# PinataFarms/DAD-3DHeads

Measured on AMD Instinct MI355X. Metric: images/sec (FLAME decode + 445-lmk projection), batch 64 @ 256^2, higher is better.
Workload: dtype f32

## Files before the change

### dad-3dheads_amd/_lib.py

```python
from __future__ import annotations

import ctypes as C
import os

_HERE = os.path.dirname(os.path.abspath(__file__))
LIB_PATH = os.environ.get("DAD3D_LIB_PATH") or os.path.join(_HERE, "libdad3d_hip.so")

OK, E_INVALID, E_HIP, E_UNSUPPORTED, E_NOMEM = range(5)
ZERO_ROTATION, TO_2D, MUTATE_PARAMS, FLIP_Z, COMPAT_CROSS_B3 = 0x1, 0x2, 0x4, 0x8, 0x10
NORMAL_ACCUMULATE = 0x1
PLAN_GET_NORMAL, PLAN_PHONG, PLAN_RENDER = 0, 1, 2
FORM_REFUSED, FORM_TABLE, FORM_LDS, FORM_GLOBAL = 0, 1, 2, 3
TEX_INDEX_CORNER, TEX_INDEX_REFERENCE = 0, 1
DTYPE_F32, DTYPE_U8 = 0, 1
EVAL_SELF_EXCLUDE, EVAL_MAX_K, EVAL_MAX_HEAD, EVAL_MAX_ANCHORS = 0x1, 8, 4096, 8
HEATMAP_RAW, HEATMAP_UINT8, HEATMAP_FLOAT = 0, 1, 2
OBJ_MAX_LINE_BYTES, OBJ_FLAG_NONFINITE, OBJ_FLAG_LARGE = 71, 0x1, 0x2
JSON_MAX_NUMBER_BYTES, JSON_MAX_LITERAL_BYTES, JSON_FLAG_NONFINITE = 23, 64, 0x1
JSON_PARSE_TILE_BYTES, JSON_PARSE_RECORD_INTS = 4096, 6
(JSON_PARSE_FLAG_GRAMMAR, JSON_PARSE_FLAG_DIGITS, JSON_PARSE_FLAG_BIG_INT, JSON_PARSE_FLAG_SUBNORMAL, JSON_PARSE_FLAG_OVERFLOW,
 JSON_PARSE_FLAG_AMBIGUOUS) = 0x1, 0x2, 0x4, 0x8, 0x10, 0x20
(ANNOTATION_FLAG_GRAMMAR, ANNOTATION_FLAG_KEYS, ANNOTATION_FLAG_SHAPE, ANNOTATION_FLAG_NUMBER, ANNOTATION_FLAG_STRING,
 ANNOTATION_FLAG_RANGE) = 0x1, 0x2, 0x4, 0x8, 0x10, 0x20
ANNOTATION_MAX_BACKSLASH_RUN, ANNOTATION_MAX_WORD_BYTES, ANNOTATION_MAX_KEY_BYTES, ANNOTATION_MAX_KEYS = 64, 32, 64, 128
# ... 40 lines not shown
        ("specular_exp", C.c_float),
        ("color_ambient", C.c_float * 3),
        ("color_directional", C.c_float * 3),
        ("light_pos", C.c_float * 3),
        ("view_pos", C.c_float * 3),
    ]


_P, _I, _U, _F = C.c_void_p, C.c_int, C.c_uint, C.c_float
SIGNATURES = {
    "dad3d_last_error": (C.c_char_p, []),
    "dad3d_clear_error": (None, []),
    "dad3d_version": (_I, []),
    "dad3d_build_info": (C.c_char_p, []),
    "dad3d_device_count": (_I, []),
    "dad3d_flame_create": (_I, [C.POINTER(FlameModelC), C.POINTER(FlameConstsC), _F, _I, C.POINTER(_P)]),
    "dad3d_flame_destroy": (None, [_P]),
    "dad3d_flame_fork": (_I, [_P, C.POINTER(_P)]),
    "dad3d_flame_num_params": (_I, [_P]),
    "dad3d_flame_num_verts": (_I, [_P]),
    "dad3d_flame_set_landmarks": (_I, [_P, _P, _I]),
    "dad3d_flame_num_landmarks": (_I, [_P]),
    "dad3d_flame_num_landmark_vertices": (_I, [_P]),
    "dad3d_flame_decode": (_I, [_P, _P, _I, _U, _P, _P, _P, _P, _P]),
    "dad3d_flame_decode_posed": (_I, [_P, _P, _I, _U, _P, _P, _P, _P]),
    "dad3d_flame_decode_backward": (_I, [_P, _I, _U, _P, _P, _P, _P, _P, _P, _P]),
    "dad3d_flame_grad_inputs": (_I, [_P, _P, _I, _P, _P]),
    "dad3d_flame_num_chain_inputs": (_I, [_P]),
    "dad3d_flame_pose_chain": (_I, [_P, _P, _I, _P, _P, _P]),
    "dad3d_flame_pose_chain_backward": (_I, [_P, _P, _I, _P, _P, _P, _P]),
    "dad3d_flame_decode_host": (_I, [_P, _P, _I, _U, _P, _P, _P, _P]),
    "dad3d_flame_readjust_params": (_I, [_P, _P, _I, _P, _F, _F, _F, _P]),
    "dad3d_flame_profile_begin": (_I, [_P, _P]),
    "dad3d_flame_profile_end": (_I, [_P, _P, C.POINTER(C.c_double), C.POINTER(_I)]),
    "dad3d_flame_select_kernel": (_I, [_P, _I]),
    "dad3d_flame_handoff_timeouts": (_I, [_P, C.POINTER(C.c_uint)]),
    "dad3d_flame_debug_trace": (_I, [_P, _P, C.c_uint64]),
    "dad3d_flame_debug_trace_entries": (C.c_uint64, [_P, _I]),
    "dad3d_mesh_create": (_I, [_P, _I, _I, _I, C.POINTER(_P)]),
    "dad3d_mesh_destroy": (None, [_P]),
    "dad3d_mesh_get_normal": (_I, [_P, _P, _P, _I, _U, _P]),
    "dad3d_mesh_get_tri_normal": (_I, [_P, _P, _P, _I, _I, _P]),
    "dad3d_mesh_get_ver_normal": (_I, [_P, _P, _P, _I, _U, _P]),
    "dad3d_mesh_rasterize": (_I, [_P, _P, _P, _P, _P, _I, _I, _I, _I, _F, _I, _P]),
    "dad3d_mesh_rasterize_triangles": (_I, [_P, _P, _P, _P, _P, _I, _I, _I, _P]),
    "dad3d_mesh_phong_light": (_I, [_P, _P, _P, _P, _I, C.POINTER(LightC), _P]),
# ... 89 lines not shown
```

### dad-3dheads_amd/csrc/capi.cpp

```cpp
#include <algorithm>
#include <cmath>
#include <cstdlib>
#include <cstring>
#include <memory>
#include <mutex>

#include "common.hpp"

namespace dad3d {

static thread_local std::string g_last_error;

void set_error(const char* fmt, ...) {
    char buf[1024];
    va_list ap;
    va_start(ap, fmt);
    vsnprintf(buf, sizeof buf, fmt, ap);
    va_end(ap);
    g_last_error = buf;
}

template <typename T>
static dad3d_status upload(T** dst, const std::vector<T>& src) {
    *dst = nullptr;
// ... 427 lines not shown

static dad3d_status ensure_basis_f16(FlameConsts* c, hipStream_t s) {
    std::lock_guard<std::mutex> lock(c->f16_mu);
    if (c->d_bpack_f16) return DAD3D_OK;
    hipStreamCaptureStatus capture = hipStreamCaptureStatusNone;
    if (s != nullptr) (void)hipStreamIsCapturing(s, &capture);
    DAD3D_REQUIRE(capture == hipStreamCaptureStatusNone, "the first fp16-split decode of a model builds its basis planes: run it once before capturing a graph");
    const size_t bytes = (size_t)c->n_tiles_pipe * kPipeKGroups * 4 * 64 * 4 * sizeof(float);
    float* d = nullptr;
    DAD3D_HIP_TRY(hipMalloc(reinterpret_cast<void**>(&d), bytes));
    dad3d_status st = launch_split_basis_f16(c->d_bpack_pipe, d, c->n_tiles_pipe, c->split_b_scale, s);
    if (st == DAD3D_OK && hipStreamSynchronize(s) != hipSuccess) {
        set_error("ensure_basis_f16: hipStreamSynchronize failed");
        st = DAD3D_E_HIP;
    }
    if (st) {
        (void)hipFree(d);
        return st;
    }
    c->d_bpack_f16 = d;
    return DAD3D_OK;
}

static dad3d_status ensure_split_scratch(dad3d_flame* h, int n_phase, hipStream_t s) {
    if (n_phase <= h->split_cap) return DAD3D_OK;
    hipStreamCaptureStatus capture = hipStreamCaptureStatusNone;
    if (s != nullptr) (void)hipStreamIsCapturing(s, &capture);
    DAD3D_REQUIRE(capture == hipStreamCaptureStatusNone,
                  "the first split-kernel decode of a handle (and the first at a larger batch) allocates: run it once before capturing a graph");
    if (h->d_split_a) h->split_retired.push_back(h->d_split_a);
    h->d_split_a = nullptr, h->split_cap = 0;
    DAD3D_HIP_TRY(hipMalloc(reinterpret_cast<void**>(&h->d_split_a), (size_t)n_phase * kSplitBlockBytes));
    DAD3D_HIP_TRY(hipMemsetAsync(h->d_split_a, 0, (size_t)n_phase * kSplitBlockBytes, s));
    h->split_cap = n_phase;
    return DAD3D_OK;
}

static int resolve_kernel(const dad3d_flame* h, int pinned, int batch, unsigned flags, bool posed) {
    const bool pipe_covers = h->c->d_bpack_pipe && !posed && !(flags & (DAD3D_COMPAT_CROSS_B3 | DAD3D_ZERO_ROTATION)) &&
                             (size_t)batch * h->n_verts * 12 < ((size_t)1 << 31) && (size_t)batch * std::max(h->lmk->n, 1) * 8 < ((size_t)1 << 31);
    if (pinned == DAD3D_KERNEL_TWO_ROLE || (pinned == DAD3D_KERNEL_AUTO && !pipe_covers)) return DAD3D_KERNEL_TWO_ROLE;
    if (pipe_covers) return pinned == DAD3D_KERNEL_AUTO ? DAD3D_KERNEL_PIPELINED : pinned;
    set_error("dad3d_flame_decode: the %s kernel does not cover this launch (model, flags or output size)",
              pinned == DAD3D_KERNEL_PIPELINED ? "pipelined" : "split");
    return -1;
}
// ... 3 lines not shown
    DAD3D_REQUIRE(h, "dad3d_flame_decode: null handle");
    DAD3D_REQUIRE(batch >= 0, "dad3d_flame_decode: negative batch");
    if (batch == 0) return DAD3D_OK;
    DAD3D_REQUIRE(params, "dad3d_flame_decode: null params");
    DAD3D_REQUIRE(!((flags & DAD3D_FLIP_Z) && (flags & DAD3D_TO_2D)), "DAD3D_FLIP_Z needs a 3-component projection");
    DAD3D_REQUIRE(!(posed && (flags & DAD3D_COMPAT_CROSS_B3)), "DAD3D_COMPAT_CROSS_B3 is inference-only (dad3d_flame_decode_posed refuses it)");
    DeviceGuard guard(h->device);
    hipStream_t s = static_cast<hipStream_t>(stream);
    const int pinned = h->kernel_choice >= 0 ? h->kernel_choice : decode_kernel_choice();
    const int kernel = resolve_kernel(h, pinned, batch, flags, posed != nullptr);
    if (kernel < 0) return DAD3D_E_UNSUPPORTED;
    const LandmarkList& L = *h->lmk;
    const int n_lmk = (lmk_xy || lmk_px) ? L.n : 0;

    const bool on_sub = L.sub && !verts3d && !proj && n_lmk && !h->d_trace && pinned != DAD3D_KERNEL_PIPELINED;
    FlameConsts* c = on_sub ? L.sub.get() : h->c.get();
    const float4* vtab = on_sub ? L.d_sub_vtab : L.d_vtab;
    const int n_verts = on_sub ? L.sub_verts : h->n_verts;

    dad3d_status st;
    if (kernel == DAD3D_KERNEL_SPLIT_BF16 || kernel == DAD3D_KERNEL_SPLIT_F16) {
        DAD3D_REQUIRE(!h->d_trace, "dad3d_flame_decode: the split kernels have no trace stamps");
        const int n_phase = (batch + kSplitRows - 1) / kSplitRows;
        st = ensure_split_scratch(h, n_phase, s);
        if (!st && kernel == DAD3D_KERNEL_SPLIT_F16) st = ensure_basis_f16(c, s);
        if (!st && kernel == DAD3D_KERNEL_SPLIT_F16 && L.sub) st = ensure_basis_f16(L.sub.get(), s);
        if (st) return st;
        SplitArgs sa{};
        sa.params = params;
        sa.bpack = c->d_bpack_pipe;
        sa.bpack_f16 = c->d_bpack_f16;
        sa.vtab = vtab;
        sa.lmk_next = L.d_next;
        sa.verts3d = verts3d;
        sa.proj = proj;
        sa.lmk_xy = lmk_xy;
        sa.lmk_px = lmk_px;
        sa.aplanes = h->d_split_a;
        sa.b_scale = c->split_b_scale;
        sa.n_params = h->lay.n_params;
        sa.batch = batch;
        sa.n_phase = n_phase;
        sa.n_tiles = c->n_tiles_pipe;
        split_chunking(sa.n_tiles, n_phase, &sa.n_chunks, &sa.phases_per_chunk);
        sa.n_verts = n_verts;
        sa.n_lmk = n_lmk;
        sa.image_size = h->image_size;
        sa.flags = flags & 0xFFu;
        st = launch_flame_decode_split(sa, kernel, s);
    } else if (kernel == DAD3D_KERNEL_PIPELINED) {
        DAD3D_REQUIRE(!h->d_trace || h->trace_capacity >= trace_entries_pipe(h), "dad3d_flame_decode: the trace buffer holds %llu entries, "
                      "this launch stamps %llu (dad3d_flame_debug_trace_entries)", (unsigned long long)h->trace_capacity,
                      (unsigned long long)trace_entries_pipe(h));
        PipeArgs pa{};
        pa.params = params;
        pa.bpack = c->d_bpack_pipe;
        pa.vtab = vtab;
        pa.lmk_next = L.d_next;
        pa.verts3d = verts3d;
        pa.proj = proj;
        pa.lmk_xy = lmk_xy;
        pa.lmk_px = lmk_px;
        pa.trace = h->d_trace;
        pa.n_params = h->lay.n_params;
        pa.batch = batch;
        pa.n_half = (batch + kPipeHalf - 1) / kPipeHalf;
        pa.n_tiles = c->n_tiles_pipe;
// ... 101 lines not shown
    if (!st) fail(hipDeviceSynchronize(), "hipDeviceSynchronize");
    if (!st && (flags & DAD3D_MUTATE_PARAMS)) fail(hipMemcpy(params, d_par, n_par * sizeof(float), hipMemcpyDeviceToHost), "hipMemcpy");
    if (!st && n_v) fail(hipMemcpy(verts3d, d_v, n_v * sizeof(float), hipMemcpyDeviceToHost), "hipMemcpy");
    if (!st && n_p) fail(hipMemcpy(proj, d_p, n_p * sizeof(float), hipMemcpyDeviceToHost), "hipMemcpy");
    if (!st && n_lx) fail(hipMemcpy(lmk_xy, d_lx, n_lx * sizeof(float), hipMemcpyDeviceToHost), "hipMemcpy");
    if (!st && n_lp) fail(hipMemcpy(lmk_px, d_lp, n_lp * sizeof(int32_t), hipMemcpyDeviceToHost), "hipMemcpy");
    (void)hipFree(d);
    return st;
}

dad3d_status dad3d_flame_readjust_params(dad3d_flame* h, float* params, int batch, const float* pads_scale,
                                         float pad_left, float pad_top, float scale, void* stream) {
    DAD3D_REQUIRE(h && batch >= 0, "dad3d_flame_readjust_params: bad argument");
    if (batch == 0) return DAD3D_OK;
    DAD3D_REQUIRE(params, "dad3d_flame_readjust_params: null params");
    DeviceGuard guard(h->device);
    return launch_readjust(params, batch, h->lay, pads_scale, pad_left, pad_top, scale, h->image_size,
                           static_cast<hipStream_t>(stream));
}

dad3d_status dad3d_flame_select_kernel(dad3d_flame* h, int which) {
    DAD3D_REQUIRE(h && which >= DAD3D_KERNEL_AUTO && which <= DAD3D_KERNEL_SPLIT_F16, "dad3d_flame_select_kernel: bad argument");
    h->kernel_choice = which;
    return DAD3D_OK;
}

dad3d_status dad3d_flame_handoff_timeouts(dad3d_flame* h, unsigned* count) {
    DAD3D_REQUIRE(h && count, "null argument");
    DeviceGuard guard(h->device);
    DAD3D_HIP_TRY(hipDeviceSynchronize());
    DAD3D_HIP_TRY(hipMemcpy(count, h->d_sync + 1, sizeof(unsigned), hipMemcpyDeviceToHost));
    return DAD3D_OK;
}

uint64_t dad3d_flame_debug_trace_entries(const dad3d_flame* h, int batch) {
    if (!h || batch <= 0) return 0;
    return std::max(trace_entries_two_role(h, batch), trace_entries_pipe(h));
}

dad3d_status dad3d_flame_debug_trace(dad3d_flame* h, unsigned long long* device_buffer, uint64_t capacity) {
    DAD3D_REQUIRE(h, "null handle");
    h->d_trace = device_buffer;
    h->trace_capacity = device_buffer ? capacity : 0;
    return DAD3D_OK;
}

// ... 1314 lines not shown
```

### dad-3dheads_amd/csrc/common.hpp

```cpp
#pragma once

#include <hip/hip_runtime.h>

#include <atomic>
#include <cstdarg>
#include <cstdint>
#include <cstdio>
#include <string>
#include <vector>

#include "../../include/dad3d.h"

namespace dad3d {

void set_error(const char* fmt, ...);

#define DAD3D_HIP_TRY(expr)                                                                      \
    do {                                                                                         \
        hipError_t e__ = (expr);                                                                 \
        if (e__ != hipSuccess) {                                                                 \
            ::dad3d::set_error("%s failed: %s (%s:%d)", #expr, hipGetErrorString(e__), __FILE__, \
                               __LINE__);                                                        \
            return DAD3D_E_HIP;                                                                  \
        }                                                                                        \
// ... 121 lines not shown
    float* params;
    const float* bpack;
    const float* bpack_f16;
    const float4* vtab;
    const int* lmk_next;
    float* verts3d;
    float* proj;
    float* lmk_xy;
    int32_t* lmk_px;
    char* aplanes;
    float b_scale;
    int n_params, batch, n_phase, n_tiles, n_verts, n_lmk;
    int n_chunks, phases_per_chunk;
    float image_size;
    unsigned flags;
};
inline void split_chunking(int n_tiles, int n_phase, int* n_chunks, int* phases_per_chunk) {
    *n_chunks = 1, *phases_per_chunk = n_phase;
    const int max_chunks = 256 / n_tiles;
    if (max_chunks < 2 || n_phase < 2) return;
    *phases_per_chunk = (n_phase + max_chunks - 1) / max_chunks;
    *n_chunks = (n_phase + *phases_per_chunk - 1) / *phases_per_chunk;
}
dad3d_status launch_flame_decode_split(const SplitArgs& a, int form, hipStream_t s);
float split_basis_scale(float max_abs);
dad3d_status launch_split_basis_f16(const float* bpack, float* bpack_f16, int n_tiles, float scale, hipStream_t s);
size_t flame_decode_split_lds_bytes();

constexpr int kBackwardConsts = 72;
struct BackwardArgs {
    const float* weights8;
    const float* consts;
    const float* posed;
    const float* g_verts3d;
    const float* g_proj;
    float* g_posed;
    float* g_consts;
    float* partials;
    int batch, n_verts, nsplit;
    float image_size;
    unsigned flags;
};
dad3d_status launch_flame_backward(const BackwardArgs& a, hipStream_t s);
constexpr int kBackwardMaxSplit = 8;

constexpr int kGradChunk = 256;
// ... 376 lines not shown
```

### dad-3dheads_amd/csrc/flame_decode_split.hip

```cpp
#pragma clang fp contract(off)
#include "common.hpp"
#include "flame_math.hpp"
#include "flame_pipe_epilogue.hpp"

#ifndef DAD3D_SPLIT_ABLATE
#define DAD3D_SPLIT_ABLATE 0
#endif

#ifndef DAD3D_SPLIT_FIN_PRIO
#define DAD3D_SPLIT_FIN_PRIO 1
#endif

namespace dad3d {

namespace {

using namespace pipe;

typedef __bf16 bf16x8 __attribute__((ext_vector_type(8)));
typedef _Float16 f16x8 __attribute__((ext_vector_type(8)));
typedef float f32x8 __attribute__((ext_vector_type(8)));

constexpr int TV = kPipeTileVerts;
constexpr int kJawCol = 3 * TV;
// ... 34 lines not shown
    static constexpr int c_off = a_off + 3 * PLN;
    static constexpr int o_off = c_off + 8 * CST;
    static constexpr int v_off = o_off + 2 * 2 * QB * OS * 4;
    static constexpr int total = v_off + TV * 16;
    static_assert(total <= 160 * 1024 && c_off % 1024 == 0 && o_off % 16 == 0 && v_off % 16 == 0, "LDS budget of one CU");
};

__device__ __forceinline__ void phase_barrier() {
    asm volatile("s_waitcnt lgkmcnt(0)\n\ts_barrier" ::: "memory");
}

template <class V>
__device__ __forceinline__ f32x8 peel(f32x8 r, V& plane) {
    plane = __builtin_convertvector(r, V);
    return r - __builtin_convertvector(plane, f32x8);
}

__device__ __forceinline__ void glds_1k(const char* gsrc_lane, char* lds_base) {
    __builtin_amdgcn_global_load_lds((const __attribute__((address_space(1))) void*)gsrc_lane, (__attribute__((address_space(3))) void*)lds_base, 16, 0, 0);
}

}

template <class S>
__global__ __launch_bounds__(256) void split_params_kernel(SplitArgs a) {
    constexpr int PLN = S::PLN, BLK = S::PLN + CST;
    const int b = blockIdx.x, t = threadIdx.x, P = a.n_params;
    if (DAD3D_SPLIT_ABLATE & 2048) return;
    const bool live = b < a.batch;
    float* prow = a.params + (size_t)min(b, a.batch - 1) * P;
    char* blk = a.aplanes + (size_t)(b / QB) * BLK;
    char* row = blk + (size_t)(b % QB) * RS;
    if ((DAD3D_SPLIT_ABLATE & 4096) && *reinterpret_cast<const volatile unsigned*>(row) != 0u) return;
    float D[9] = {0.f, 0.f, 0.f, 0.f, 0.f, 0.f, 0.f, 0.f, 0.f};
    if (t >= 192) {
        const float jaw[3] = {prow[kNumBeta], prow[kNumBeta + 1], prow[kNumBeta + 2]};
        rodrigues_minus_identity_lean(jaw, D);
    }
    if (t < 208) {
        const int k0 = 2 * t;
        float x = 0.f, y = 0.f;
        if (k0 < kNumBeta) x = prow[k0], y = prow[k0 + 1];
        const float tail[16] = {D[0], D[1], D[2], D[3], D[4], D[5], D[6], D[7], D[8], 1.0f, 0.f, 0.f, 0.f, 0.f, 0.f, 0.f};
#pragma unroll
        for (int i = 0; i < 8; ++i)
            if (t - kNumBeta / 2 == i) x = tail[2 * i], y = tail[2 * i + 1];
        if (!live || (DAD3D_SPLIT_ABLATE & 16384)) x = y = 0.f;
        const int g = k0 >> 5, h = (k0 >> 4) & 1, q = (k0 >> 2) & 3, i = k0 & 3;
        const int pos = 32 * g + 8 * q + 4 * h + i;
        float rx = x * S::kScaleA, ry = y * S::kScaleA;
#pragma unroll
        for (int pl = 0; pl < S::NPL; ++pl) {
            const typename S::elem hx = (typename S::elem)rx, hy = (typename S::elem)ry;
            rx = rx - (float)hx, ry = ry - (float)hy;
            const unsigned packed = (unsigned)__builtin_bit_cast(unsigned short, hx) | ((unsigned)__builtin_bit_cast(unsigned short, hy) << 16);
            *reinterpret_cast<unsigned*>(row + (size_t)pl * QB * RS + 2 * pos) = packed;
        }
    } else if (t < 208 + 4 * S::NPL) {
        const int pl = (t - 208) >> 2, w = (t - 208) & 3;
        *reinterpret_cast<unsigned*>(row + (size_t)pl * QB * RS + 832 + 4 * w) = 0u;
    } else if (t == 255 && !(DAD3D_SPLIT_ABLATE & 8192)) {
        float* c = reinterpret_cast<float*>(blk + PLN + (size_t)(b % QB) * 96);
        *reinterpret_cast<float4*>(c) = float4{D[0], D[1], D[2], D[3]};
        *reinterpret_cast<float4*>(c + 4) = float4{D[4], D[5], D[6], D[7]};
        c[8] = D[8];
    }
    if (t == 0 && !(DAD3D_SPLIT_ABLATE & 8192)) {
        const float rot6[6] = {prow[403], prow[404], prow[405], prow[406], prow[407], prow[408]};
        const float sp1 = prow[412] + 1.0f, tx = prow[409], ty = prow[410];
        float G[9];
        rot6_to_matrix_lean(rot6, G);
        const float s = sp1 < 1e-8f ? 1e-8f : sp1;
        float* c = reinterpret_cast<float*>(blk + PLN + (size_t)(b % QB) * 96);
        c[9] = G[0], c[10] = G[1], c[11] = G[2];
        *reinterpret_cast<float4*>(c + 12) = float4{G[3], G[4], G[5], G[6]};
        const float hh = a.image_size * 0.5f;
        *reinterpret_cast<float4*>(c + 16) = float4{G[7], G[8], s * hh, (tx + 1.0f) * hh};
        *reinterpret_cast<float4*>(c + 20) = float4{(ty + 1.0f) * hh, hh, 0.f, 0.f};
        if ((a.flags & DAD3D_MUTATE_PARAMS) && live) prow[kNumBeta + 11] = 0.0f;
    }
}

template <class S, bool TO2D, bool WB>
__global__ __launch_bounds__(64 * (5 + S::kFinishers), (5 + S::kFinishers + 3) / 4) void flame_decode_split_kernel(SplitArgs a) {
    typedef typename S::vec8 vec8;
    constexpr int NPL = S::NPL, PLN = S::PLN, BLK = S::PLN + CST;
    extern __shared__ __attribute__((aligned(1024))) char smem[];
    char* abuf = smem + Lds<S>::a_off;
    char* cring = smem + Lds<S>::c_off;
    float* otile = reinterpret_cast<float*>(smem + Lds<S>::o_off);
    float4* vt_lds = reinterpret_cast<float4*>(smem + Lds<S>::v_off);

    const int tid = threadIdx.x, lane = tid & 63;
    const int wave = __builtin_amdgcn_readfirstlane(tid >> 6);
    const int n_work = a.n_tiles * a.n_chunks;
    const int xcd = blockIdx.x & 7, slot = blockIdx.x >> 3, big = n_work & 7, per = n_work >> 3;
    const int work = xcd < big ? xcd * (per + 1) + slot : big * (per + 1) + (xcd - big) * per + slot;
    const int tile = work / a.n_chunks, chunk = work - tile * a.n_chunks, v0 = tile * TV;
    const int pb = chunk * a.phases_per_chunk;
    const int NP = min(a.phases_per_chunk, a.n_phase - pb), B = a.batch;
    if (NP <= 0) return;

    if (wave == 4) {
        auto stage = [&](int p) {
            const char* src = a.aplanes + (size_t)(pb + p) * BLK + 16 * lane;
            char* dst = abuf + (p % 3) * PLN;
#if defined(DAD3D_SPLIT_NO_GLDS)
#pragma unroll 1
            for (int i0 = 0; i0 < PLN / 1024; i0 += 8) {
                f32x4 v[8];
#pragma unroll
                for (int i = 0; i < 8; ++i) v[i] = *reinterpret_cast<const f32x4*>(src + 1024 * (i0 + i));
#pragma unroll
                for (int i = 0; i < 8; ++i) *reinterpret_cast<f32x4*>(dst + 1024 * (i0 + i) + 16 * lane) = v[i];
            }
            for (int i = 0; i < CST / 1024; ++i)
                *reinterpret_cast<f32x4*>(cring + (p & 7) * CST + 1024 * i + 16 * lane) = *reinterpret_cast<const f32x4*>(src + PLN + 1024 * i);
#else
#pragma unroll 8
            for (int i = 0; i < PLN / 1024; ++i) glds_1k(src + 1024 * i, dst + 1024 * i);
#pragma unroll
            for (int i = 0; i < CST / 1024; ++i) glds_1k(src + PLN + 1024 * i, cring + (p & 7) * CST + 1024 * i);
#endif
        };
        constexpr int kStageOps = PLN / 1024 + CST / 1024;
        static_assert(kStageOps <= 63, "vmcnt is a 6-bit counter");
        if (lane < TV) vt_lds[lane] = a.vtab[min(v0 + lane, a.n_verts - 1)];
        asm volatile("s_waitcnt vmcnt(0)" ::: "memory");
        stage(0);
        if (NP > 1) {
            stage(1);
            asm volatile("s_waitcnt vmcnt(%0)" ::"n"(kStageOps) : "memory");
        } else {
            asm volatile("s_waitcnt vmcnt(0)" ::: "memory");
        }
        phase_barrier();
#pragma unroll 1
        for (int p = 0; p < NP; ++p) {
            if (p + 2 < NP && (!(DAD3D_SPLIT_ABLATE & 2) || p < 1)) {
                stage(p + 2);
                asm volatile("s_waitcnt vmcnt(%0)" ::"n"(kStageOps) : "memory");
            } else {
                asm volatile("s_waitcnt vmcnt(0)" ::: "memory");
            }
            phase_barrier();
        }
        phase_barrier();
        return;
    }
    const unsigned nl = (unsigned)a.n_lmk;
    EpiCtx cx;
// ... 29 lines not shown
    struct Call {
        float4 k0, k1, k2, k3, k4, k5;
        float j0[3], j1[3], e0[3], e1[3];
    };
    auto load_call = [&](int q, const Geo& g, Call& t) {
        const float4* cp = reinterpret_cast<const float4*>(cring + (q & 7) * CST + g.cp_off);
        t.k0 = cp[0], t.k1 = cp[1], t.k2 = cp[2], t.k3 = cp[3], t.k4 = cp[4], t.k5 = cp[5];
        const float* ot = otile + (q & 1) * (2 * QB * OS);
#pragma unroll
        for (int k = 0; k < 3; ++k) {
            t.j0[k] = ot[g.jt_off + k], t.j1[k] = ot[QB * OS + g.jt_off + k];
            t.e0[k] = ot[g.ot_off + k], t.e1[k] = ot[QB * OS + g.ot_off + k];
        }
    };
    auto math_call = [&](const Geo& g, const Call& t) {
        if (DAD3D_SPLIT_ABLATE & 512) return VertexOut{t.e0[0] + t.k0.x, t.e0[1] + t.k1.x, t.e0[2] + t.k2.x, t.e1[0] + t.k3.x + t.j0[0], t.e1[1] + t.k4.x + t.j0[1], t.e1[2] + t.k5.x + t.j1[0]};
        return vertex_math_folded(cx, t.k0, t.k1, t.k2, t.k3, t.k4, t.k5, t.j0[0] + t.j1[0], t.j0[1] + t.j1[1], t.j0[2] + t.j1[2], t.e0[0] + t.e1[0],
                                  t.e0[1] + t.e1[1], t.e0[2] + t.e1[2], g.vt.x, g.vt.y);
    };
    auto store_call = [&](int q, const Geo& g, const VertexOut& o) {
        const int b = (pb + q) * QB + g.i;
        const bool live = b < B && g.vlive && !((DAD3D_SPLIT_ABLATE & 256) && o.ox != 12345.678f);
        const unsigned row0 = (unsigned)((pb + q) * QB) * (unsigned)a.n_verts;
        vertex_store_at<TO2D, WB ? 0 : DAD3D_PIPE_STORE_AUX>(cx, rs3, rsp, o, __float_as_int(g.vt.z), __float_as_int(g.vt.w), live && a.verts3d != nullptr, live && a.proj != nullptr,
                              live && nl > 0 && __float_as_int(g.vt.z) >= 0, g.off3 + row0 * 12u, g.offp + row0 * kPB, (unsigned)b * nl);
    };
    auto finish_one = [&](int q, const Geo& g) {
        Call t;
        load_call(q, g, t);
        store_call(q, g, math_call(g, t));
    };
    auto finish_two = [&](int q, const Geo& ga, const Geo& gb) {
        Call ta, tb;
        load_call(q, ga, ta);
        load_call(q, gb, tb);
        const VertexOut oa = math_call(ga, ta), ob = math_call(gb, tb);
        store_call(q, ga, oa);
        store_call(q, gb, ob);
    };

    if (wave > 4) {
        const int fj = wave - 5;
        __builtin_amdgcn_s_setprio(DAD3D_SPLIT_FIN_PRIO);
        phase_barrier();
        constexpr bool kTwoCalls = S::kFinishers == 3;
        const Geo ga = make_geo(fj), gb = make_geo(kTwoCalls && fj < 2 ? fj + 3 : fj);
#pragma unroll 1
        for (int p = 0; p < NP; ++p) {
            if (p >= 2 && !(DAD3D_SPLIT_ABLATE & 1)) {
                if (kTwoCalls && fj < 2) finish_two(p - 2, ga, gb);
                else finish_one(p - 2, ga);
            }
            phase_barrier();
        }
        if (NP >= 2 && !(DAD3D_SPLIT_ABLATE & 1)) finish_one(NP - 2, ga);
        phase_barrier();
        if (!(DAD3D_SPLIT_ABLATE & 1)) finish_one(NP - 1, ga);
        return;
    }

    const int kh = wave >> 1, ch = wave & 1, c0 = 2 * ch + kh, c1 = 2 * ch + 1 - kh, gbase = 6 * kh;
    const float4* bsrc = reinterpret_cast<const float4*>(S::kScaled ? a.bpack_f16 : a.bpack) + (size_t)tile * kPipeKGroups * 256 + lane;
    float4 raw[6][2][2], rawt[2][2];
#pragma unroll
    for (int sl = 0; sl < 6; ++sl)
#pragma unroll
        for (int cb = 0; cb < 2; ++cb)
#pragma unroll
            for (int h = 0; h < 2; ++h) {
                raw[sl][cb][h] = bsrc[(size_t)((2 * (gbase + sl) + h) * 4 + (cb ? c1 : c0)) * 64];
                __builtin_amdgcn_sched_barrier(0);
            }
#pragma unroll
    for (int cb = 0; cb < 2; ++cb)
#pragma unroll
// ... 76 lines not shown
    const long long clk0 = clock64(), wall0 = wall_clock64();
#endif
    read_frags(0, gbase, af);
    if constexpr (S::kScaled) {
#pragma unroll
        for (int sl = 0; sl < 6; ++sl) planes(raw[sl][0][0], raw[sl][0][1], bp[sl][0]), planes(raw[sl][1][0], raw[sl][1][1], bp[sl][1]);
        planes(rawt[0][0], rawt[0][1], bt[0]), planes(rawt[1][0], rawt[1][1], bt[1]);
#pragma unroll 1
        for (int p = 0; p < NP; ++p) phase(p, std::false_type{});
    } else {
        phase(0, std::true_type{});
#pragma unroll 1
        for (int p = 1; p < NP; ++p) phase(p, std::false_type{});
    }
    if (S::kFinishers == 3 && wave < 2 && !(DAD3D_SPLIT_ABLATE & 1)) {
        const Geo g = make_geo(3 + wave);
        if (NP >= 2) finish_one(NP - 2, g);
        phase_barrier();
        finish_one(NP - 1, g);
        return;
    }
    phase_barrier();
#if defined(DAD3D_SPLIT_CLOCKS)
    if (tile == 17 && tid == 130) {
        unsigned* cnt = reinterpret_cast<unsigned*>(a.aplanes + PLN + 1536);
        const unsigned n = atomicAdd(cnt, 1u);
        const long long dc = clock64() - clk0, dw = wall_clock64() - wall0;
        if ((n & 255u) == 255u) printf("CLK n_phase %d cycles %lld ticks %lld MHz %.0f cycles/phase %.0f\n", NP, dc, dw, (double)dc / (dw * 10.0) * 1e3, (double)dc / NP);
    }
#endif
}

__global__ __launch_bounds__(256) void split_basis_f16_kernel(const float4* src, float4* dst, int n_tiles, float scale) {
    const size_t i = (size_t)blockIdx.x * 256 + threadIdx.x;
    const size_t n = (size_t)n_tiles * kSplitKGroups * 256;
    if (i >= n) return;
    const size_t t = i / (kSplitKGroups * 256), g = (i / 256) % kSplitKGroups, r = i % 256;
    const size_t i0 = (t * kPipeKGroups + 2 * g) * 256 + r, i1 = i0 + 256;
    const float4 lo = src[i0], hi = src[i1];
    float e[8] = {lo.x, lo.y, lo.z, lo.w, hi.x, hi.y, hi.z, hi.w};
    f16x8 h1, h2;
#pragma unroll
    for (int k = 0; k < 8; ++k) {
        const float x = e[k] * scale;
        h1[k] = (_Float16)x;
        h2[k] = (_Float16)(x - (float)h1[k]);
    }
    dst[i0] = __builtin_bit_cast(float4, h1), dst[i1] = __builtin_bit_cast(float4, h2);
}

dad3d_status launch_split_basis_f16(const float* bpack, float* bpack_f16, int n_tiles, float scale, hipStream_t s) {
    static_assert(kPipeKGroups == 2 * kSplitKGroups, "two MFMA groups of 16 k per 16-bit group of 32");
    const size_t n = (size_t)n_tiles * kSplitKGroups * 256;
    hipLaunchKernelGGL(split_basis_f16_kernel, dim3((unsigned)((n + 255) / 256)), dim3(256), 0, s, reinterpret_cast<const float4*>(bpack),
                       reinterpret_cast<float4*>(bpack_f16), n_tiles, scale);
    DAD3D_HIP_TRY(hipGetLastError());
    return DAD3D_OK;
}

size_t flame_decode_split_lds_bytes() { return (size_t)Lds<Bf16x3>::total; }

namespace {
template <class S>
dad3d_status launch_split(const SplitArgs& a, hipStream_t s, PerDeviceOnce& attr_done) {
    const int dev = PerDeviceOnce::current();
    const size_t lds = (size_t)Lds<S>::total;
    if (!attr_done.done(dev)) {
        for (const void* k : {reinterpret_cast<const void*>(&flame_decode_split_kernel<S, true, false>),
                              reinterpret_cast<const void*>(&flame_decode_split_kernel<S, false, false>),
                              reinterpret_cast<const void*>(&flame_decode_split_kernel<S, true, true>),
                              reinterpret_cast<const void*>(&flame_decode_split_kernel<S, false, true>)})
            DAD3D_HIP_TRY(hipFuncSetAttribute(k, hipFuncAttributeMaxDynamicSharedMemorySize, (int)lds));
        attr_done.set(dev);
    }
    hipLaunchKernelGGL(split_params_kernel<S>, dim3(a.n_phase * kSplitRows), dim3(256), 0, s, a);
    const bool to2d = (a.flags & DAD3D_TO_2D) || !a.proj, wb = a.batch >= S::kWriteBackFrom;
    const dim3 grid(a.n_tiles * a.n_chunks), block(64 * (5 + S::kFinishers));
    if (to2d && wb) hipLaunchKernelGGL((flame_decode_split_kernel<S, true, true>), grid, block, lds, s, a);
    else if (to2d) hipLaunchKernelGGL((flame_decode_split_kernel<S, true, false>), grid, block, lds, s, a);
    else if (wb) hipLaunchKernelGGL((flame_decode_split_kernel<S, false, true>), grid, block, lds, s, a);
    else hipLaunchKernelGGL((flame_decode_split_kernel<S, false, false>), grid, block, lds, s, a);
    DAD3D_HIP_TRY(hipGetLastError());
    return DAD3D_OK;
}
}

dad3d_status launch_flame_decode_split(const SplitArgs& a, int form, hipStream_t s) {
    static PerDeviceOnce attr_bf16, attr_f16;
    if (form == DAD3D_KERNEL_SPLIT_F16) return launch_split<F16x2>(a, s, attr_f16);
    return launch_split<Bf16x3>(a, s, attr_bf16);
}

float split_basis_scale(float max_abs) {
    float s = 1.0f;
    while (s < 16777216.0f && max_abs * (s * 2.0f) <= 16384.0f) s *= 2.0f;
    return s;
}

}
```

### include/dad3d.h

```cpp
#ifndef DAD3D_H_
#define DAD3D_H_

#include <stddef.h>
#include <stdint.h>

#ifndef DAD3D_EXPORT
#define DAD3D_EXPORT __attribute__((visibility("default")))
#endif

#ifdef __cplusplus
extern "C" {
#endif

#define DAD3D_VERSION 100

typedef enum dad3d_status {
    DAD3D_OK = 0,
    DAD3D_E_INVALID = 1,
    DAD3D_E_HIP = 2,
    DAD3D_E_UNSUPPORTED = 3,
    DAD3D_E_NOMEM = 4
} dad3d_status;

DAD3D_EXPORT const char* dad3d_last_error(void);
// ... 18 lines not shown
typedef struct dad3d_flame_consts {
    int32_t shape, expression, jaw, rotation, eyeballs, neck, translation, scale;
} dad3d_flame_consts;

typedef struct dad3d_flame dad3d_flame;

#define DAD3D_ZERO_ROTATION 0x1u
#define DAD3D_TO_2D 0x2u
#define DAD3D_MUTATE_PARAMS 0x4u
#define DAD3D_FLIP_Z 0x8u
#define DAD3D_COMPAT_CROSS_B3 0x10u

DAD3D_EXPORT dad3d_status dad3d_flame_create(const dad3d_flame_model* model, const dad3d_flame_consts* consts, float image_size,
                                int device, dad3d_flame** out);
DAD3D_EXPORT void dad3d_flame_destroy(dad3d_flame* h);
DAD3D_EXPORT dad3d_status dad3d_flame_fork(dad3d_flame* parent, dad3d_flame** out);

DAD3D_EXPORT int dad3d_flame_num_params(const dad3d_flame* h);
DAD3D_EXPORT int dad3d_flame_num_verts(const dad3d_flame* h);

DAD3D_EXPORT dad3d_status dad3d_flame_set_landmarks(dad3d_flame* h, const int64_t* indices, int n);
DAD3D_EXPORT int dad3d_flame_num_landmarks(const dad3d_flame* h);
DAD3D_EXPORT int dad3d_flame_num_landmark_vertices(const dad3d_flame* h);

DAD3D_EXPORT dad3d_status dad3d_flame_decode(dad3d_flame* h, float* params, int batch, unsigned flags, float* verts3d, float* proj,
                                float* lmk_xy, int32_t* lmk_px, void* stream);

DAD3D_EXPORT dad3d_status dad3d_flame_decode_posed(dad3d_flame* h, float* params, int batch, unsigned flags, float* verts3d, float* proj,
                                      float* posed, void* stream);

DAD3D_EXPORT dad3d_status dad3d_flame_decode_backward(dad3d_flame* h, int batch, unsigned flags, const float* consts, const float* posed,
                                         const float* grad_verts3d, const float* grad_proj, float* grad_posed,
                                         float* grad_consts, void* stream);

#define DAD3D_GRAD_INPUTS_MAX_BATCH 96
DAD3D_EXPORT dad3d_status dad3d_flame_grad_inputs(dad3d_flame* h, const float* grad_posed, int batch, float* grad_inputs, void* stream);

DAD3D_EXPORT int dad3d_flame_num_chain_inputs(const dad3d_flame* h);
DAD3D_EXPORT dad3d_status dad3d_flame_pose_chain(dad3d_flame* h, const float* params, int batch, float* inputs, float* consts, void* stream);
DAD3D_EXPORT dad3d_status dad3d_flame_pose_chain_backward(dad3d_flame* h, const float* params, int batch, const float* grad_inputs,
                                             const float* grad_consts, float* grad_params, void* stream);

DAD3D_EXPORT dad3d_status dad3d_flame_decode_host(dad3d_flame* h, float* params, int batch, unsigned flags, float* verts3d,
                                     float* proj, float* lmk_xy, int32_t* lmk_px);

DAD3D_EXPORT dad3d_status dad3d_flame_readjust_params(dad3d_flame* h, float* params, int batch, const float* pads_scale,
// ... 245 lines not shown
```

Baseline: 5.030 million.

## Fuse param splitting into split decode kernel for landmark-only small-batch path

For landmark-only decodes on the landmark subset with at most two phases per workgroup, the separate split_params_kernel launch is removed. Each decode workgroup now reads the raw parameters and builds the bf16/f16 plane images and per-row constants itself, using the staging and finisher waves as producers. This cuts one kernel launch and the global round trip through the A-plane scratch, at the cost of every tile redundantly recomputing the parameter split. It is on by default and can be turned off with an environment variable, and a plan query API is added.

Result: no change. 5.037 million (median of 4 runs) (+0.1%).

```diff
diff --git a/dad-3dheads_amd/_lib.py b/dad-3dheads_amd/_lib.py
--- a/dad-3dheads_amd/_lib.py
+++ b/dad-3dheads_amd/_lib.py
@@ -86,6 +86,7 @@
     "dad3d_flame_set_landmarks": (_I, [_P, _P, _I]),
     "dad3d_flame_num_landmarks": (_I, [_P]),
     "dad3d_flame_num_landmark_vertices": (_I, [_P]),
+    "dad3d_flame_landmark_plan": (_I, [_P, _I, C.POINTER(_I), C.POINTER(_I), C.POINTER(_I), C.POINTER(_I), C.POINTER(_I)]),
     "dad3d_flame_decode": (_I, [_P, _P, _I, _U, _P, _P, _P, _P, _P]),
     "dad3d_flame_decode_posed": (_I, [_P, _P, _I, _U, _P, _P, _P, _P]),
     "dad3d_flame_decode_backward": (_I, [_P, _I, _U, _P, _P, _P, _P, _P, _P, _P]),
diff --git a/dad-3dheads_amd/csrc/capi.cpp b/dad-3dheads_amd/csrc/capi.cpp
--- a/dad-3dheads_amd/csrc/capi.cpp
+++ b/dad-3dheads_amd/csrc/capi.cpp
@@ -473,6 +473,14 @@
     return DAD3D_OK;
 }
 
+static bool split_lmk_one_launch() {
+    static const bool on = [] {
+        const char* e = getenv("DAD3D_SPLIT_LMK_ONE_LAUNCH");
+        return !(e && e[0] == '0');
+    }();
+    return on;
+}
+
 static dad3d_status ensure_split_scratch(dad3d_flame* h, int n_phase, hipStream_t s) {
     if (n_phase <= h->split_cap) return DAD3D_OK;
     hipStreamCaptureStatus capture = hipStreamCaptureStatusNone;
@@ -522,7 +530,10 @@
     if (kernel == DAD3D_KERNEL_SPLIT_BF16 || kernel == DAD3D_KERNEL_SPLIT_F16) {
         DAD3D_REQUIRE(!h->d_trace, "dad3d_flame_decode: the split kernels have no trace stamps");
         const int n_phase = (batch + kSplitRows - 1) / kSplitRows;
-        st = ensure_split_scratch(h, n_phase, s);
+        int n_chunks = 1, phases_per_chunk = n_phase;
+        split_chunking(c->n_tiles_pipe, n_phase, &n_chunks, &phases_per_chunk);
+        const bool one_launch = on_sub && phases_per_chunk <= kSplitOneLaunchPhases && split_lmk_one_launch();
+        st = one_launch ? DAD3D_OK : ensure_split_scratch(h, n_phase, s);
         if (!st && kernel == DAD3D_KERNEL_SPLIT_F16) st = ensure_basis_f16(c, s);
         if (!st && kernel == DAD3D_KERNEL_SPLIT_F16 && L.sub) st = ensure_basis_f16(L.sub.get(), s);
         if (st) return st;
@@ -536,13 +547,13 @@
         sa.proj = proj;
         sa.lmk_xy = lmk_xy;
         sa.lmk_px = lmk_px;
-        sa.aplanes = h->d_split_a;
+        sa.aplanes = one_launch ? nullptr : h->d_split_a;
         sa.b_scale = c->split_b_scale;
         sa.n_params = h->lay.n_params;
         sa.batch = batch;
         sa.n_phase = n_phase;
         sa.n_tiles = c->n_tiles_pipe;
-        split_chunking(sa.n_tiles, n_phase, &sa.n_chunks, &sa.phases_per_chunk);
+        sa.n_chunks = n_chunks, sa.phases_per_chunk = phases_per_chunk;
         sa.n_verts = n_verts;
         sa.n_lmk = n_lmk;
         sa.image_size = h->image_size;
@@ -690,6 +701,29 @@
 dad3d_status dad3d_flame_select_kernel(dad3d_flame* h, int which) {
     DAD3D_REQUIRE(h && which >= DAD3D_KERNEL_AUTO && which <= DAD3D_KERNEL_SPLIT_F16, "dad3d_flame_select_kernel: bad argument");
     h->kernel_choice = which;
+    return DAD3D_OK;
+}
+
+dad3d_status dad3d_flame_landmark_plan(dad3d_flame* h, int batch, int* kernel, int* tiles, int* chunks, int* rows_per_chunk, int* launches) {
+    DAD3D_REQUIRE(h && batch > 0 && kernel && tiles && chunks && rows_per_chunk && launches, "dad3d_flame_landmark_plan: bad argument");
+    const int pinned = h->kernel_choice >= 0 ? h->kernel_choice : decode_kernel_choice();
+    const int k = resolve_kernel(h, pinned, batch, 0u, false);
+    if (k < 0) return DAD3D_E_UNSUPPORTED;
+    const LandmarkList& L = *h->lmk;
+    const bool on_sub = L.sub && L.n && !h->d_trace && pinned != DAD3D_KERNEL_PIPELINED && k != DAD3D_KERNEL_TWO_ROLE;
+    *kernel = k;
+    *tiles = k == DAD3D_KERNEL_TWO_ROLE ? h->n_tiles : on_sub ? L.sub->n_tiles_pipe : h->c->n_tiles_pipe;
+    *chunks = 1, *rows_per_chunk = batch, *launches = 1;
+    if (k == DAD3D_KERNEL_SPLIT_BF16 || k == DAD3D_KERNEL_SPLIT_F16) {
+        int ppc = 0;
+        split_chunking(*tiles, (batch + kSplitRows - 1) / kSplitRows, chunks, &ppc);
+        *rows_per_chunk = ppc * kSplitRows;
+        *launches = on_sub && ppc <= kSplitOneLaunchPhases && split_lmk_one_launch() ? 1 : 2;
+    } else if (k == DAD3D_KERNEL_PIPELINED && !h->d_trace) {
+        int chunk_half = 0, wg = 0;
+        pipe_chunking(*tiles, (batch + kPipeHalf - 1) / kPipeHalf, &chunk_half, chunks, &wg);
+        if (chunk_half > 0) *rows_per_chunk = chunk_half * kPipeHalf;
+    }
     return DAD3D_OK;
 }
 
diff --git a/dad-3dheads_amd/csrc/common.hpp b/dad-3dheads_amd/csrc/common.hpp
--- a/dad-3dheads_amd/csrc/common.hpp
+++ b/dad-3dheads_amd/csrc/common.hpp
@@ -167,6 +167,7 @@
     *phases_per_chunk = (n_phase + max_chunks - 1) / max_chunks;
     *n_chunks = (n_phase + *phases_per_chunk - 1) / *phases_per_chunk;
 }
+constexpr int kSplitOneLaunchPhases = 2;
 dad3d_status launch_flame_decode_split(const SplitArgs& a, int form, hipStream_t s);
 float split_basis_scale(float max_abs);
 dad3d_status launch_split_basis_f16(const float* bpack, float* bpack_f16, int n_tiles, float scale, hipStream_t s);
diff --git a/dad-3dheads_amd/csrc/flame_decode_split.hip b/dad-3dheads_amd/csrc/flame_decode_split.hip
--- a/dad-3dheads_amd/csrc/flame_decode_split.hip
+++ b/dad-3dheads_amd/csrc/flame_decode_split.hip
@@ -80,6 +80,79 @@
 
 }
 
+__device__ __forceinline__ void load_jaw(const float* prow, float (&jaw)[3]) {
+    jaw[0] = prow[kNumBeta], jaw[1] = prow[kNumBeta + 1], jaw[2] = prow[kNumBeta + 2];
+}
+__device__ __forceinline__ void load_pose(const float* prow, float (&v)[9]) {
+#pragma unroll
+    for (int i = 0; i < 8; ++i) v[i] = prow[403 + i];
+    v[8] = prow[412];
+}
+__device__ __forceinline__ void jaw_feature(const float (&jaw)[3], float (&D)[9]) {
+    rodrigues_minus_identity_lean(jaw, D);
+}
+__device__ __forceinline__ void store_jaw_constants(const float (&D)[9], float* c) {
+    *reinterpret_cast<float4*>(c) = float4{D[0], D[1], D[2], D[3]};
+    *reinterpret_cast<float4*>(c + 4) = float4{D[4], D[5], D[6], D[7]};
+    c[8] = D[8];
+}
+__device__ __forceinline__ void store_pose_constants(const float (&v)[9], float image_size, float* c) {
+    const float rot6[6] = {v[0], v[1], v[2], v[3], v[4], v[5]};
+    const float sp1 = v[8] + 1.0f, tx = v[6], ty = v[7];
+    float G[9];
+    rot6_to_matrix_lean(rot6, G);
+    const float s = sp1 < 1e-8f ? 1e-8f : sp1;
+    c[9] = G[0], c[10] = G[1], c[11] = G[2];
+    *reinterpret_cast<float4*>(c + 12) = float4{G[3], G[4], G[5], G[6]};
+    const float hh = image_size * 0.5f;
+    *reinterpret_cast<float4*>(c + 16) = float4{G[7], G[8], s * hh, (tx + 1.0f) * hh};
+    *reinterpret_cast<float4*>(c + 20) = float4{(ty + 1.0f) * hh, hh, 0.f, 0.f};
+}
+__device__ __forceinline__ void beta_pair(const float* prow, int t, float& x, float& y) {
+    const int k0 = 2 * t;
+    if (k0 < kNumBeta) x = prow[k0], y = prow[k0 + 1];
+}
+__device__ __forceinline__ void tail_pair(const float (&D)[9], int j, float& x, float& y) {
+    const float tail[16] = {D[0], D[1], D[2], D[3], D[4], D[5], D[6], D[7], D[8], 1.0f, 0.f, 0.f, 0.f, 0.f, 0.f, 0.f};
+#pragma unroll
+    for (int i = 0; i < 8; ++i)
+        if (j == i) x = tail[2 * i], y = tail[2 * i + 1];
+}
+template <class S>
+__device__ __forceinline__ void split_element(float x, typename S::elem (&h)[S::NPL]) {
+    float r = x * S::kScaleA;
+#pragma unroll
+    for (int pl = 0; pl < S::NPL; ++pl) {
+        h[pl] = (typename S::elem)r;
+        r = r - (float)h[pl];
+    }
+}
+template <class S>
+__device__ __forceinline__ void store_pair_planes(float x, float y, int t, char* row) {
+    const int k0 = 2 * t, g = k0 >> 5, h = (k0 >> 4) & 1, q = (k0 >> 2) & 3, i = k0 & 3;
+    const int pos = 32 * g + 8 * q + 4 * h + i;
+    typename S::elem hx[S::NPL], hy[S::NPL];
+    split_element<S>(x, hx), split_element<S>(y, hy);
+#pragma unroll
+    for (int pl = 0; pl < S::NPL; ++pl) {
+        const unsigned packed = (unsigned)__builtin_bit_cast(unsigned short, hx[pl]) | ((unsigned)__builtin_bit_cast(unsigned short, hy[pl]) << 16);
+        *reinterpret_cast<unsigned*>(row + (size_t)pl * QB * RS + 2 * pos) = packed;
+    }
+}
+template <class S>
+__device__ __forceinline__ void store_oct_planes(const float (&e)[8], char* dst) {
+    typename S::vec8 v[S::NPL];
+#pragma unroll
+    for (int i = 0; i < 8; ++i) {
+        typename S::elem h[S::NPL];
+        split_element<S>(e[i], h);
+#pragma unroll
+        for (int pl = 0; pl < S::NPL; ++pl) v[pl][i] = h[pl];
+    }
+#pragma unroll
+    for (int pl = 0; pl < S::NPL; ++pl) *reinterpret_cast<typename S::vec8*>(dst + (size_t)pl * QB * RS) = v[pl];
+}
+
 template <class S>
 __global__ __launch_bounds__(256) void split_params_kernel(SplitArgs a) {
     constexpr int PLN = S::PLN, BLK = S::PLN + CST;
@@ -92,55 +165,32 @@
     if ((DAD3D_SPLIT_ABLATE & 4096) && *reinterpret_cast<const volatile unsigned*>(row) != 0u) return;
     float D[9] = {0.f, 0.f, 0.f, 0.f, 0.f, 0.f, 0.f, 0.f, 0.f};
     if (t >= 192) {
-        const float jaw[3] = {prow[kNumBeta], prow[kNumBeta + 1], prow[kNumBeta + 2]};
-        rodrigues_minus_identity_lean(jaw, D);
+        float jaw[3];
+        load_jaw(prow, jaw);
+        jaw_feature(jaw, D);
     }
     if (t < 208) {
-        const int k0 = 2 * t;
         float x = 0.f, y = 0.f;
-        if (k0 < kNumBeta) x = prow[k0], y = prow[k0 + 1];
-        const float tail[16] = {D[0], D[1], D[2], D[3], D[4], D[5], D[6], D[7], D[8], 1.0f, 0.f, 0.f, 0.f, 0.f, 0.f, 0.f};
-#pragma unroll
-        for (int i = 0; i < 8; ++i)
-            if (t - kNumBeta / 2 == i) x = tail[2 * i], y = tail[2 * i + 1];
+        beta_pair(prow, t, x, y);
+        tail_pair(D, t - kNumBeta / 2, x, y);
         if (!live || (DAD3D_SPLIT_ABLATE & 16384)) x = y = 0.f;
-        const int g = k0 >> 5, h = (k0 >> 4) & 1, q = (k0 >> 2) & 3, i = k0 & 3;
-        const int pos = 32 * g + 8 * q + 4 * h + i;
-        float rx = x * S::kScaleA, ry = y * S::kScaleA;
-#pragma unroll
-        for (int pl = 0; pl < S::NPL; ++pl) {
-            const typename S::elem hx = (typename S::elem)rx, hy = (typename S::elem)ry;
-            rx = rx - (float)hx, ry = ry - (float)hy;
-            const unsigned packed = (unsigned)__builtin_bit_cast(unsigned short, hx) | ((unsigned)__builtin_bit_cast(unsigned short, hy) << 16);
-            *reinterpret_cast<unsigned*>(row + (size_t)pl * QB * RS + 2 * pos) = packed;
-        }
+        store_pair_planes<S>(x, y, t, row);
     } else if (t < 208 + 4 * S::NPL) {
         const int pl = (t - 208) >> 2, w = (t - 208) & 3;
         *reinterpret_cast<unsigned*>(row + (size_t)pl * QB * RS + 832 + 4 * w) = 0u;
     } else if (t == 255 && !(DAD3D_SPLIT_ABLATE & 8192)) {
-        float* c = reinterpret_cast<float*>(blk + PLN + (size_t)(b % QB) * 96);
-        *reinterpret_cast<float4*>(c) = float4{D[0], D[1], D[2], D[3]};
-        *reinterpret_cast<float4*>(c + 4) = float4{D[4], D[5], D[6], D[7]};
-        c[8] = D[8];
+        store_jaw_constants(D, reinterpret_cast<float*>(blk + PLN + (size_t)(b % QB) * 96));
     }
     if (t == 0 && !(DAD3D_SPLIT_ABLATE & 8192)) {
-        const float rot6[6] = {prow[403], prow[404], prow[405], prow[406], prow[407], prow[408]};
-        const float sp1 = prow[412] + 1.0f, tx = prow[409], ty = prow[410];
-        float G[9];
-        rot6_to_matrix_lean(rot6, G);
-        const float s = sp1 < 1e-8f ? 1e-8f : sp1;
-        float* c = reinterpret_cast<float*>(blk + PLN + (size_t)(b % QB) * 96);
-        c[9] = G[0], c[10] = G[1], c[11] = G[2];
-        *reinterpret_cast<float4*>(c + 12) = float4{G[3], G[4], G[5], G[6]};
-        const float hh = a.image_size * 0.5f;
-        *reinterpret_cast<float4*>(c + 16) = float4{G[7], G[8], s * hh, (tx + 1.0f) * hh};
-        *reinterpret_cast<float4*>(c + 20) = float4{(ty + 1.0f) * hh, hh, 0.f, 0.f};
+        float v[9];
+        load_pose(prow, v);
+        store_pose_constants(v, a.image_size, reinterpret_cast<float*>(blk + PLN + (size_t)(b % QB) * 96));
         if ((a.flags & DAD3D_MUTATE_PARAMS) && live) prow[kNumBeta + 11] = 0.0f;
     }
 }
 
-template <class S, bool TO2D, bool WB>
-__global__ __launch_bounds__(64 * (5 + S::kFinishers), (5 + S::kFinishers + 3) / 4) void flame_decode_split_kernel(SplitArgs a) {
+template <class S, bool TO2D, bool WB, bool ONE>
+__device__ __forceinline__ void split_tile(const SplitArgs& a) {
     typedef typename S::vec8 vec8;
     constexpr int NPL = S::NPL, PLN = S::PLN, BLK = S::PLN + CST;
     extern __shared__ __attribute__((aligned(1024))) char smem[];
@@ -159,6 +209,89 @@
     const int NP = min(a.phases_per_chunk, a.n_phase - pb), B = a.batch;
     if (NP <= 0) return;
 
+    constexpr int kOcts = QB * 12 * 4, kItems = 2 + kOcts / 64, kProducers = 1 + S::kFinishers;
+    static_assert(kOcts % 64 == 0 && kProducers >= 2, "whole items; the two constants' items on two producers");
+    constexpr int kShareN = (kItems + kProducers - 1) / kProducers;
+    struct Raw {
+        float e[kShareN][8], jaw[3], pose[9], tb[16];
+    };
+    auto request_share = [&](int p, int pi, Raw& w) {
+        constexpr int stride = kProducers, end = kItems;
+        const int it0 = pi;
+        const int row0 = (pb + p) * QB, P = a.n_params;
+        const float* crow = a.params + (size_t)min(row0 + (lane & (QB - 1)), B - 1) * P;
+#pragma unroll
+        for (int u = 0; u < kShareN; ++u) {
+            const int it = it0 + u * stride;
+#pragma unroll
+            for (int i = 0; i < 8; ++i) w.e[u][i] = 0.f;
+            if (it >= end) continue;
+            if (u == 0 && it == 0) {
+                if (lane < QB) {
+                    load_jaw(crow, w.jaw);
+#pragma unroll
+                    for (int i = 0; i < 16; ++i) w.tb[i] = crow[384 + i];
+                }
+            } else if (u == 0 && it == 1) {
+                if (lane < QB) load_pose(crow, w.pose);
+            } else {
+                const int j = 64 * (it - 2) + lane, r = j / 48, rem = j - 48 * r, kb = 32 * (rem >> 2) + 4 * (rem & 3);
+                if (row0 + r < B) {
+                    const float* prow = a.params + (size_t)(row0 + r) * P + kb;
+#pragma unroll
+                    for (int i = 0; i < 4; ++i) w.e[u][i] = prow[i], w.e[u][4 + i] = prow[16 + i];
+                }
+            }
+        }
+    };
+    auto split_share = [&](int p, int pi, const Raw& w) {
+        constexpr int stride = kProducers, end = kItems;
+        const int it0 = pi;
+        char* img = abuf + (p % 3) * PLN;
+        const int row0 = (pb + p) * QB, rc = lane & (QB - 1);
+        float* c = reinterpret_cast<float*>(cring + (p & 7) * CST + rc * 96);
+#pragma unroll
+        for (int u = 0; u < kShareN; ++u) {
+            const int it = it0 + u * stride;
+            if (it >= end) continue;
+            if (u == 0 && it == 0) {
+                if (lane < QB) {
+                    float D[9];
+                    jaw_feature(w.jaw, D);
+                    store_jaw_constants(D, c);
+                    const bool live = row0 + rc < B;
+#pragma unroll
+                    for (int q = 0; q < 4; ++q) {
+                        float e[8] = {w.tb[4 * q], w.tb[4 * q + 1], w.tb[4 * q + 2], w.tb[4 * q + 3], 0.f, 0.f, 0.f, 0.f};
+                        tail_pair(D, 2 * q, e[4], e[5]);
+                        tail_pair(D, 2 * q + 1, e[6], e[7]);
+#pragma unroll
+                        for (int i = 0; i < 8; ++i) e[i] = live ? e[i] : 0.f;
+                        store_oct_planes<S>(e, img + rc * RS + 64 * 12 + 16 * q);
+                    }
+                }
+            } else if (u == 0 && it == 1) {
+                if (lane < QB) {
+                    store_pose_constants(w.pose, a.image_size, c);
+                    if ((a.flags & DAD3D_MUTATE_PARAMS) && row0 + rc < B && tile == 0)
+                        a.params[(size_t)(row0 + rc) * a.n_params + kNumBeta + 11] = 0.0f;
+                }
+            } else {
+                const int j = 64 * (it - 2) + lane, r = j / 48, rem = j - 48 * r;
+                store_oct_planes<S>(w.e[u], img + r * RS + 16 * rem);
+            }
+        }
+    };
+    auto produce_launch = [&](int pi, auto&& behind_s0) {
+        Raw w0, w1;
+        request_share(0, pi, w0);
+        if (NP > 1) request_share(1, pi, w1);
+        split_share(0, pi, w0);
+        phase_barrier();
+        behind_s0();
+        if (NP > 1) split_share(1, pi, w1);
+    };
+
     if (wave == 4) {
         auto stage = [&](int p) {
             const char* src = a.aplanes + (size_t)(pb + p) * BLK + 16 * lane;
@@ -185,6 +318,12 @@
         static_assert(kStageOps <= 63, "vmcnt is a 6-bit counter");
         if (lane < TV) vt_lds[lane] = a.vtab[min(v0 + lane, a.n_verts - 1)];
         asm volatile("s_waitcnt vmcnt(0)" ::: "memory");
+        if constexpr (ONE) {
+            produce_launch(0, [] {});
+            for (int p = 0; p < NP; ++p) phase_barrier();
+            phase_barrier();
+            return;
+        }
         stage(0);
         if (NP > 1) {
             stage(1);
@@ -260,7 +399,7 @@
         const int b = (pb + q) * QB + g.i;
         const bool live = b < B && g.vlive && !((DAD3D_SPLIT_ABLATE & 256) && o.ox != 12345.678f);
         const unsigned row0 = (unsigned)((pb + q) * QB) * (unsigned)a.n_verts;
-        vertex_store_at<TO2D, WB ? 0 : DAD3D_PIPE_STORE_AUX>(cx, rs3, rsp, o, __float_as_int(g.vt.z), __float_as_int(g.vt.w), live && a.verts3d != nullptr, live && a.proj != nullptr,
+        vertex_store_at<TO2D, WB ? 0 : DAD3D_PIPE_STORE_AUX>(cx, rs3, rsp, o, __float_as_int(g.vt.z), __float_as_int(g.vt.w), !ONE && live && a.verts3d != nullptr, !ONE && live && a.proj != nullptr,
                               live && nl > 0 && __float_as_int(g.vt.z) >= 0, g.off3 + row0 * 12u, g.offp + row0 * kPB, (unsigned)b * nl);
     };
     auto finish_one = [&](int q, const Geo& g) {
@@ -280,15 +419,24 @@
     if (wave > 4) {
         const int fj = wave - 5;
         __builtin_amdgcn_s_setprio(DAD3D_SPLIT_FIN_PRIO);
-        phase_barrier();
         constexpr bool kTwoCalls = S::kFinishers == 3;
-        const Geo ga = make_geo(fj), gb = make_geo(kTwoCalls && fj < 2 ? fj + 3 : fj);
-#pragma unroll 1
-        for (int p = 0; p < NP; ++p) {
+        Geo ga, gb;
+        auto geos = [&] { ga = make_geo(fj), gb = make_geo(kTwoCalls && fj < 2 ? fj + 3 : fj); };
+        auto finish_window = [&](int p) {
             if (p >= 2 && !(DAD3D_SPLIT_ABLATE & 1)) {
                 if (kTwoCalls && fj < 2) finish_two(p - 2, ga, gb);
                 else finish_one(p - 2, ga);
             }
+        };
+        if constexpr (ONE) {
+            produce_launch(fj + 1, geos);
+        } else {
+            phase_barrier();
+            geos();
+        }
+#pragma unroll 1
+        for (int p = 0; p < NP; ++p) {
+            finish_window(p);
             phase_barrier();
         }
         if (NP >= 2 && !(DAD3D_SPLIT_ABLATE & 1)) finish_one(NP - 2, ga);
@@ -411,13 +559,22 @@
     }
     phase_barrier();
 #if defined(DAD3D_SPLIT_CLOCKS)
-    if (tile == 17 && tid == 130) {
+    if (!ONE && tile == 17 && tid == 130) {
         unsigned* cnt = reinterpret_cast<unsigned*>(a.aplanes + PLN + 1536);
         const unsigned n = atomicAdd(cnt, 1u);
         const long long dc = clock64() - clk0, dw = wall_clock64() - wall0;
         if ((n & 255u) == 255u) printf("CLK n_phase %d cycles %lld ticks %lld MHz %.0f cycles/phase %.0f\n", NP, dc, dw, (double)dc / (dw * 10.0) * 1e3, (double)dc / NP);
     }
 #endif
+}
+
+template <class S, bool TO2D, bool WB>
+__global__ __launch_bounds__(64 * (5 + S::kFinishers), (5 + S::kFinishers + 3) / 4) void flame_decode_split_kernel(SplitArgs a) {
+    split_tile<S, TO2D, WB, false>(a);
+}
+template <class S, bool TO2D>
+__global__ __launch_bounds__(64 * (5 + S::kFinishers), (5 + S::kFinishers + 3) / 4) void flame_decode_split_lmk_kernel(SplitArgs a) {
+    split_tile<S, TO2D, false, true>(a);
 }
 
 __global__ __launch_bounds__(256) void split_basis_f16_kernel(const float4* src, float4* dst, int n_tiles, float scale) {
@@ -458,13 +615,25 @@
         for (const void* k : {reinterpret_cast<const void*>(&flame_decode_split_kernel<S, true, false>),
                               reinterpret_cast<const void*>(&flame_decode_split_kernel<S, false, false>),
                               reinterpret_cast<const void*>(&flame_decode_split_kernel<S, true, true>),
-                              reinterpret_cast<const void*>(&flame_decode_split_kernel<S, false, true>)})
+                              reinterpret_cast<const void*>(&flame_decode_split_kernel<S, false, true>),
+                              reinterpret_cast<const void*>(&flame_decode_split_lmk_kernel<S, true>),
+                              reinterpret_cast<const void*>(&flame_decode_split_lmk_kernel<S, false>)})
             DAD3D_HIP_TRY(hipFuncSetAttribute(k, hipFuncAttributeMaxDynamicSharedMemorySize, (int)lds));
         attr_done.set(dev);
     }
-    hipLaunchKernelGGL(split_params_kernel<S>, dim3(a.n_phase * kSplitRows), dim3(256), 0, s, a);
     const bool to2d = (a.flags & DAD3D_TO_2D) || !a.proj, wb = a.batch >= S::kWriteBackFrom;
     const dim3 grid(a.n_tiles * a.n_chunks), block(64 * (5 + S::kFinishers));
+    if (!a.aplanes) {
+        if (a.verts3d || a.proj || !a.n_lmk || a.phases_per_chunk > kSplitOneLaunchPhases) {
+            set_error("launch_flame_decode_split: the one-launch form writes landmark outputs only, at most %d phases per workgroup", kSplitOneLaunchPhases);
+            return DAD3D_E_INVALID;
+        }
+        if (a.flags & DAD3D_TO_2D) hipLaunchKernelGGL((flame_decode_split_lmk_kernel<S, true>), grid, block, lds, s, a);
+        else hipLaunchKernelGGL((flame_decode_split_lmk_kernel<S, false>), grid, block, lds, s, a);
+        DAD3D_HIP_TRY(hipGetLastError());
+        return DAD3D_OK;
+    }
+    hipLaunchKernelGGL(split_params_kernel<S>, dim3(a.n_phase * kSplitRows), dim3(256), 0, s, a);
     if (to2d && wb) hipLaunchKernelGGL((flame_decode_split_kernel<S, true, true>), grid, block, lds, s, a);
     else if (to2d) hipLaunchKernelGGL((flame_decode_split_kernel<S, true, false>), grid, block, lds, s, a);
     else if (wb) hipLaunchKernelGGL((flame_decode_split_kernel<S, false, true>), grid, block, lds, s, a);
diff --git a/include/dad3d.h b/include/dad3d.h
--- a/include/dad3d.h
+++ b/include/dad3d.h
@@ -64,6 +64,8 @@
 DAD3D_EXPORT dad3d_status dad3d_flame_set_landmarks(dad3d_flame* h, const int64_t* indices, int n);
 DAD3D_EXPORT int dad3d_flame_num_landmarks(const dad3d_flame* h);
 DAD3D_EXPORT int dad3d_flame_num_landmark_vertices(const dad3d_flame* h);
+DAD3D_EXPORT dad3d_status dad3d_flame_landmark_plan(dad3d_flame* h, int batch, int* kernel, int* tiles, int* chunks, int* rows_per_chunk,
+                                       int* launches);
 
 DAD3D_EXPORT dad3d_status dad3d_flame_decode(dad3d_flame* h, float* params, int batch, unsigned flags, float* verts3d, float* proj,
                                 float* lmk_xy, int32_t* lmk_px, void* stream);
```
